# FudanCVL/SynFMC

Measured on AMD Instinct MI355X. Metric: denoising steps/sec, 16x320x512 bf16 U-Net+CMC+OMC, higher is better.
Workload: dtype bf16; 1 GPU; 16x320x512 clip, CFG batch 2, full-width 3D U-Net (1.39B params, random init) + Camera Adapter (CMC) + Object Motion Control (OMC) features, DDIM step; configs/obj.yaml shapes; 1 clip per GPU; frames=16, height=320, width=512, hip_graph=True, fp8_temporal_attention=False, parallelism=dp1 (independent clips, no collective)

## Files before the change

synfmc_amd/csrc/spatial_attn.hip:

```cpp
#include "attn_common.h"
#include <cstdlib>

namespace {

constexpr int SA_WAVES = 4;
constexpr int SA_BQ = 32 * SA_WAVES;
constexpr bool SA_PREFETCH_DEFAULT = true;
constexpr int SA_BK = 64;
constexpr float LOG2E = 1.4426950408889634f;

struct SAParams {
    const void* q; const void* k; const void* v; void* o; float* lse;
    int B, H, Sq, Skv, D;
    int64_t qbs, qrs, kbs, krs, obs, ors;
    int kv_batch_div;
    float scale_log2;
    int nqblk;
    int xcd_remap;
};

constexpr float REF_LIMIT = 64.f;
#ifndef SA_DBG
#define SA_DBG 0
#endif
// ... 826 lines not shown
#pragma unroll
        for (int kb = 0; kb < NKB; ++kb) {
#pragma unroll
            for (int r = 0; r < 16; ++r) s[kb][r] = 0.f;
#pragma unroll
            for (int ks = 0; ks < NKS; ++ks) s[kb] = __builtin_amdgcn_mfma_f32_32x32x16_bf16(kf[kb][ks], qf[ks], s[kb], 0, 0, 0);
        }
        float mx = -INFINITY;
#pragma unroll
        for (int kb = 0; kb < NKB; ++kb)
#pragma unroll
            for (int r = 0; r < 16; ++r) {
                const int key = kb * 32 + (r & 3) + 8 * (r >> 2) + 4 * half;
                if (key >= P.Skv) s[kb][r] = -INFINITY;
                mx = fmaxf(mx, s[kb][r]);
            }
        mx = fmaxf(mx, __shfl_xor(mx, 32, 64));
        f32x16 oacc[NDT];
#pragma unroll
        for (int dt = 0; dt < NDT; ++dt)
#pragma unroll
            for (int r = 0; r < 16; ++r) oacc[dt][r] = 0.f;
#pragma unroll
        for (int kb = 0; kb < NKB; ++kb) {
            float pv[16];
#pragma unroll
            for (int r = 0; r < 16; ++r) pv[r] = __builtin_amdgcn_exp2f(s[kb][r] - mx);
#pragma unroll
            for (int s2 = 0; s2 < 2; ++s2) {
                float p8[8];
#pragma unroll
                for (int i = 0; i < 8; ++i) p8[i] = pv[s2 * 8 + i];
                Frag<bf16_t> pf;
                p_frag(p8, pf);
#pragma unroll
                for (int dt = 0; dt < NDT; ++dt) oacc[dt] = __builtin_amdgcn_mfma_f32_32x32x16_bf16(vf[kb][s2][dt], pf.hi, oacc[dt], 0, 0, 0);
            }
        }
        const float l_tot = __shfl(oacc[NDT - 1][15], l31 + 32, 64);
        const float inv = 1.f / l_tot;
        const int b = kvb * P.kv_batch_div + u / nq32, q = (u - (u / nq32) * nq32) * 32 + l31;
        bf16_t* orow = (bf16_t*)P.o + (int64_t)b * P.obs + (int64_t)q * P.ors + h * D;
#pragma unroll
        for (int dt = 0; dt < NDT; ++dt)
#pragma unroll
            for (int g = 0; g < 4; ++g) {
                const int d = dt * 32 + 8 * g + 4 * half;
                if (d < D)
                    store4<bf16_t>(orow + d, oacc[dt][4 * g] * inv, oacc[dt][4 * g + 1] * inv, oacc[dt][4 * g + 2] * inv, oacc[dt][4 * g + 3] * inv);
            }
        if (P.lse && half == 0) P.lse[((int64_t)b * P.H + h) * P.Sq + q] = mx * 0.6931471805599453f + logf(l_tot);
#pragma unroll
        for (int ks = 0; ks < NKS; ++ks) qf[ks] = qn[ks];
    }
}

inline int sa_xattn_env() {
    static const int v = fmc_env_int("FMC_SA_XATTN", 1);
    return v;
}
inline bool xattn40_ok(const SAParams& P) {
    return P.D == 40 && P.H == 8 && P.Skv <= 96 && P.Skv >= 1 && P.Sq % 32 == 0 && P.B % P.kv_batch_div == 0 && sa_xattn_env() != 0;
}
inline void launch_xattn40(const SAParams& P, hipStream_t st) {
    const int nkvb = P.B / P.kv_batch_div, nq32 = P.Sq / 32, units = P.kv_batch_div * nq32;
    int per = fmc_cu_count() / nkvb;
    if (per < 1) per = 1;
    if (per > units) per = units;
    const size_t lds = (size_t)8 * 96 * XA_VP * 2;
    fmc_launch<xattn40_kernel>(dim3((unsigned)(per * nkvb)), dim3(512), lds, st, P, nq32, units, nkvb);
}

template <int NB>
__global__ __launch_bounds__(320, 1) void sa_small160_kernel(const SAParams P) {
    typedef bf16_t T;
    constexpr int NKS = 10, NDT = 5, KP = NKS * 16 + 8, VPR = sa_vr_pitch<NDT>(), CH = 20, NKEY = NB * 32, NT = 320;
    extern __shared__ __attribute__((aligned(16))) unsigned char smem_raw[];
    T* Ks = reinterpret_cast<T*>(smem_raw);
    T* Vr = Ks + NKEY * KP;
    const int tid = threadIdx.x, lane = tid & 63, wave = tid >> 6;
    const int half = lane >> 5, l31 = lane & 31;
    const int bh = blockIdx.x / P.nqblk, qblk = blockIdx.x - bh * P.nqblk;
    const int b = bh / P.H, h = bh - b * P.H;
    const T* qg = (const T*)P.q + (int64_t)b * P.qbs + (int64_t)h * 160;
    const T* kg = (const T*)P.k + (int64_t)(b / P.kv_batch_div) * P.kbs + (int64_t)h * 160;
    const T* vg = (const T*)P.v + (int64_t)(b / P.kv_batch_div) * P.kbs + (int64_t)h * 160;
    T* og = (T*)P.o + (int64_t)b * P.obs + (int64_t)h * 160;

    constexpr int NSLOT = NKEY * CH / NT;
    static_assert(NKEY * CH % NT == 0, "whole chunks per thread");
    u32x4 kreg[NSLOT], vreg[NSLOT];
    auto gload = [&](const T* base, u32x4 (&reg)[NSLOT]) {
#pragma unroll
        for (int j = 0; j < NSLOT; ++j) {
            const int c = tid + j * NT, row = c / CH, ch = c - row * CH;
            reg[j] = *reinterpret_cast<const u32x4*>(base + (int64_t)(row < P.Skv ? row : P.Skv - 1) * P.krs + ch * 8);
        }
    };
    auto lstore = [&](T* dst, int pitch, const u32x4 (&reg)[NSLOT]) {
#pragma unroll
        for (int j = 0; j < NSLOT; ++j) {
            const int c = tid + j * NT, row = c / CH, ch = c - row * CH;
            *reinterpret_cast<u32x4*>(dst + row * pitch + ch * 8) = reg[j];
        }
    };
    gload(kg, kreg);
    const int qrow = (qblk * 5 + wave) * 32 + l31;
    const bool active = (qblk * 5 + wave) * 32 < P.Sq;
    u32x4 qraw[NKS];
    {
        const T* qp = qg + (int64_t)(qrow < P.Sq ? qrow : P.Sq - 1) * P.qrs + half * 8;
#pragma unroll
        for (int ks = 0; ks < NKS; ++ks) qraw[ks] = *reinterpret_cast<const u32x4*>(qp + ks * 16);
    }
    gload(vg, vreg);
    lstore(Ks, KP, kreg);
    Frag<T> qf[1][NKS];
#pragma unroll
    for (int ks = 0; ks < NKS; ++ks) {
        float qv[8];
#pragma unroll
        for (int i = 0; i < 4; ++i) {
            qv[2 * i] = __uint_as_float(qraw[ks][i] << 16) * P.scale_log2;
            qv[2 * i + 1] = __uint_as_float(qraw[ks][i] & 0xffff0000u) * P.scale_log2;
        }
        p_frag(qv, qf[0][ks]);
    }
    __syncthreads();

    Frag<T> pf[NB][2];
    float m = 0.f, l_run = 0.f;
    if (active) {
        f32x16 s[NB];
#pragma unroll
        for (int blk = 0; blk < NB; ++blk)
#pragma unroll
            for (int r = 0; r < 16; ++r) s[blk][r] = 0.f;
#pragma unroll
        for (int ks = 0; ks < NKS; ++ks)
#pragma unroll
            for (int blk = 0; blk < NB; ++blk) {
                Frag<T> kf;
                make_frag<T>(Ks + (blk * 32 + l31) * KP + ks * 16 + half * 8, kf);
                mma32(kf, qf[0][ks], s[blk]);
            }
        float mx = -INFINITY;
#pragma unroll
        for (int blk = 0; blk < NB; ++blk) {
            if ((blk + 1) * 32 > P.Skv) {
#pragma unroll
                for (int r = 0; r < 16; ++r)
                    if (blk * 32 + (r & 3) + 8 * (r >> 2) + 4 * half >= P.Skv) s[blk][r] = -INFINITY;
            }
            mx = fold_max(s[blk], mx);
        }
        m = fmaxf(mx, __shfl_xor(mx, 32, 64));
#pragma unroll
        for (int blk = 0; blk < NB; ++blk) {
            float p[16];
#pragma unroll
            for (int r = 0; r < 16; ++r) {
                p[r] = __builtin_amdgcn_exp2f(s[blk][r] - m);
                l_run += p[r];
            }
#pragma unroll
            for (int s2 = 0; s2 < 2; ++s2) {
                float p8[8];
#pragma unroll
                for (int i = 0; i < 8; ++i) p8[i] = p[s2 * 8 + i];
                p_frag(p8, pf[blk][s2]);
            }
        }
    }
    lstore(Vr, VPR, vreg);
    __syncthreads();
    if (!active) return;

    f32x16 oacc[NDT];
#pragma unroll
    for (int dt = 0; dt < NDT; ++dt)
#pragma unroll
        for (int r = 0; r < 16; ++r) oacc[dt][r] = 0.f;
#pragma unroll
    for (int blk = 0; blk < NB; ++blk)
#pragma unroll
        for (int s2 = 0; s2 < 2; ++s2)
#pragma unroll
            for (int dt = 0; dt < NDT; ++dt) {
                const T* vp = Vr + (blk * 32 + s2 * 16 + half * 4 + ((l31 & 15) >> 2)) * VPR + dt * 32 + (l31 >> 4) * 16 + (l31 & 3) * 4;
                union { bf16x8 v; sa_s4 hh[2]; } rr;
                rr.hh[0] = lds_tr16(vp);
                rr.hh[1] = lds_tr16(vp + 8 * VPR);
                Frag<T> vf;
                vf.hi = rr.v;
                mma32(vf, pf[blk][s2], oacc[dt]);
            }
    const float l_tot = l_run + __shfl_xor(l_run, 32, 64);
    const float inv = 1.f / l_tot;
    if (qrow < P.Sq) {
        T* orow = og + (int64_t)qrow * P.ors;
#pragma unroll
        for (int dt = 0; dt < NDT; ++dt)
#pragma unroll
            for (int g = 0; g < 4; ++g)
                store4<T>(orow + dt * 32 + 8 * g + 4 * half, oacc[dt][4 * g] * inv, oacc[dt][4 * g + 1] * inv,
                          oacc[dt][4 * g + 2] * inv, oacc[dt][4 * g + 3] * inv);
        if (P.lse && half == 0) P.lse[((int64_t)b * P.H + h) * P.Sq + qrow] = m * 0.6931471805599453f + logf(l_tot);
    }
}

template <int NW>
__device__ __forceinline__ void sa_big80_body(const SAParams& P) {
    typedef bf16_t T;
    constexpr int NKS = 5, NDT = 3, KP = NKS * 16 + 8, VPR = sa_vr_pitch<NDT>(), CH = 10, BKT = NW == 5 ? 160 : 320, NBLK = BKT / 32, NT = 64 * NW;
    extern __shared__ __attribute__((aligned(16))) unsigned char smem_raw[];
    T* Ks = reinterpret_cast<T*>(smem_raw);
    T* Vr = Ks + BKT * KP;
    const int tid = threadIdx.x, lane = tid & 63, wave = tid >> 6;
    const int half = lane >> 5, l31 = lane & 31;
    int bh, qblk;
    {
        const int id = blockIdx.x;
        if (P.xcd_remap == 2) {
            const int xcd = id & 7, within = id >> 3, per_b = P.H * P.nqblk, rem = within % per_b;
            bh = ((within / per_b) * 8 + xcd) * P.H + rem / P.nqblk;
            qblk = rem % P.nqblk;
        } else {
            bh = id / P.nqblk;
            qblk = id - bh * P.nqblk;
        }
    }
    const int b = bh / P.H, h = bh - b * P.H;
    const T* qg = (const T*)P.q + (int64_t)b * P.qbs + (int64_t)h * 80;
    const T* kg = (const T*)P.k + (int64_t)(b / P.kv_batch_div) * P.kbs + (int64_t)h * 80;
    const T* vg = (const T*)P.v + (int64_t)(b / P.kv_batch_div) * P.kbs + (int64_t)h * 80;
    T* og = (T*)P.o + (int64_t)b * P.obs + (int64_t)h * 80;

    constexpr int NSLOT = (BKT * CH + NT - 1) / NT;
    u32x4 kreg[NSLOT], vreg[NSLOT];
    auto gload = [&](int kv0) {
#pragma unroll
        for (int j = 0; j < NSLOT; ++j) {
            const int c = min(tid + j * NT, BKT * CH - 1), row = c / CH, ch = c - row * CH;
            const int kv = kv0 + row < P.Skv ? kv0 + row : P.Skv - 1;
            kreg[j] = *reinterpret_cast<const u32x4*>(kg + (int64_t)kv * P.krs + ch * 8);
            vreg[j] = *reinterpret_cast<const u32x4*>(vg + (int64_t)kv * P.krs + ch * 8);
        }
    };
    auto lstore = [&]() {
#pragma unroll
        for (int j = 0; j < NSLOT; ++j) {
            const int c = min(tid + j * NT, BKT * CH - 1), row = c / CH, ch = c - row * CH;
            *reinterpret_cast<u32x4*>(Ks + row * KP + ch * 8) = kreg[j];
            *reinterpret_cast<u32x4*>(Vr + row * VPR + ch * 8) = vreg[j];
        }
    };
    gload(0);
    const int qrow = (qblk * NW + wave) * 32 + l31;
    const bool active = (qblk * NW + wave) * 32 < P.Sq;
    Frag<T> qf[1][NKS];
    {
        const T* qp = qg + (int64_t)(qrow < P.Sq ? qrow : P.Sq - 1) * P.qrs + half * 8;
        u32x4 qraw[NKS];
#pragma unroll
        for (int ks = 0; ks < NKS; ++ks) qraw[ks] = *reinterpret_cast<const u32x4*>(qp + ks * 16);
#pragma unroll
        for (int ks = 0; ks < NKS; ++ks) {
            float qv[8];
#pragma unroll
            for (int i = 0; i < 4; ++i) {
                qv[2 * i] = __uint_as_float(qraw[ks][i] << 16) * P.scale_log2;
                qv[2 * i + 1] = __uint_as_float(qraw[ks][i] & 0xffff0000u) * P.scale_log2;
            }
            p_frag(qv, qf[0][ks]);
        }
    }
    for (int c = tid; c < BKT * 2; c += NT)
        *reinterpret_cast<u32x4*>(Vr + (c >> 1) * VPR + 80 + (c & 1) * 8) = u32x4{0u, 0u, 0u, (c & 1) ? 0x3f800000u : 0u};
    lstore();
    __syncthreads();

    const int ntiles = (P.Skv + BKT - 1) / BKT;
    float m_ref[1];
    f32x16 negm[1];
    {
        f32x16 zero16;
#pragma unroll
        for (int r = 0; r < 16; ++r) zero16[r] = 0.f;
        const float mx = fold_max(qk_block<T, NKS, false>(Ks, qf[0], zero16, 0, 0, P.Skv, l31, half), -INFINITY);
        m_ref[0] = fmaxf(mx, __shfl_xor(mx, 32, 64));
#pragma unroll
        for (int r = 0; r < 16; ++r) negm[0][r] = -m_ref[0];
    }
    f32x16 oacc[1][NDT];
    float l_run[1];
    for (int pass = 0; pass < 2; ++pass) {
        float worst[1] = {-INFINITY};
#pragma unroll
        for (int dt = 0; dt < NDT; ++dt)
#pragma unroll
            for (int r = 0; r < 16; ++r) oacc[0][dt][r] = 0.f;
        l_run[0] = 0.f;
        for (int tile = 0; tile < ntiles; ++tile) {
#ifndef SA_BIG_DBG
#define SA_BIG_DBG 0
#endif
            if ((tile > 0 || pass > 0) && SA_BIG_DBG != 2) {
                gload(tile * BKT);
                __syncthreads();
                lstore();
                __syncthreads();
            }
            if (active && SA_BIG_DBG != 1) {
                const int nblk = min(NBLK, (P.Skv - tile * BKT) >> 5);
                if (NW == 8 && nblk == NBLK) {
                    f32x16 s[2][1];
                    qk_scores<T, NKS, 1, false>(Ks, qf, negm, s[0], 0, l31, half);
#pragma unroll
                    for (int sb = 0; sb < NBLK; ++sb) {
                        if (sb + 1 < NBLK) qk_scores<T, NKS, 1, false>(Ks, qf, negm, s[(sb + 1) & 1], sb + 1, l31, half);
                        softmax_pv_perq<T, NKS, 1, true>(Vr, s[sb & 1], oacc, worst, l_run, sb, l31, half);
                    }
                } else {
#pragma unroll 1
                    for (int sb = 0; sb < nblk; ++sb)
                        attn_block<T, NKS, 1, false, false, true>(Ks, Vr, qf, oacc, negm, worst, l_run, sb, tile * BKT + sb * 32, P.Skv, l31, half);
                }
            }
        }
        const bool bad = active && worst[0] > REF_LIMIT;
        if (!__syncthreads_or(bad)) break;
        m_ref[0] += fmaxf(worst[0], __shfl_xor(worst[0], 32, 64));
#pragma unroll
        for (int r = 0; r < 16; ++r) negm[0][r] = -m_ref[0];
    }
    if (!active) return;
    const float l_tot = __shfl(oacc[0][NDT - 1][15], l31 + 32, 64);
    const float inv = 1.f / l_tot;
    if (qrow < P.Sq) {
        T* orow = og + (int64_t)qrow * P.ors;
#pragma unroll
        for (int dt = 0; dt < NDT; ++dt)
#pragma unroll
            for (int g = 0; g < 4; ++g) {
                const int d = dt * 32 + 8 * g + 4 * half;
                if (d < 80)
                    store4<T>(orow + d, oacc[0][dt][4 * g] * inv, oacc[0][dt][4 * g + 1] * inv, oacc[0][dt][4 * g + 2] * inv, oacc[0][dt][4 * g + 3] * inv);
            }
        if (P.lse && half == 0) P.lse[((int64_t)b * P.H + h) * P.Sq + qrow] = m_ref[0] * 0.6931471805599453f + logf(l_tot);
    }
}

__global__ __launch_bounds__(640, 1) void sa_big80_kernel_w10(const SAParams P) { sa_big80_body<10>(P); }
__global__ __launch_bounds__(512, 1) void sa_big80_kernel_w8(const SAParams P) { sa_big80_body<8>(P); }
__global__ __launch_bounds__(320, 3) void sa_big80_kernel_w5(const SAParams P) { sa_big80_body<5>(P); }

inline bool sa_big80_ok(const SAParams& P) {
    static const bool on = fmc_env_int("FMC_SA_BIG80", 1) != 0;
    return on && P.D == 80 && P.Skv % 32 == 0 && P.Skv >= 256 && P.Sq >= 160;
}
inline void launch_sa_big80(const SAParams& Pin, hipStream_t st) {
    SAParams P = Pin;
    static const int nw = [] { const int v = fmc_env_int("FMC_SA_BIG80_WAVES", 10); return v == 8 || v == 5 ? v : 10; }();
    P.nqblk = (P.Sq + 32 * nw - 1) / (32 * nw);
    if (P.xcd_remap != 2) P.xcd_remap = 0;
    const size_t lds = (size_t)(nw == 5 ? 160 : 320) * (5 * 16 + 8 + sa_vr_pitch<3>()) * 2;
    if (nw == 5) fmc_launch<sa_big80_kernel_w5>(dim3((unsigned)(P.B * P.H * P.nqblk)), dim3(320), lds, st, P);
    else if (nw == 8) fmc_launch<sa_big80_kernel_w8>(dim3((unsigned)(P.B * P.H * P.nqblk)), dim3(512), lds, st, P);
    else fmc_launch<sa_big80_kernel_w10>(dim3((unsigned)(P.B * P.H * P.nqblk)), dim3(640), lds, st, P);
}

inline bool sa_small_ok(const SAParams& P) {
    static const bool on = fmc_env_int("FMC_SA_SMALL", 1) != 0;
    return on && P.D == 160 && P.Skv <= 160;
}
template <int NB>
void launch_sa_small_nb(const SAParams& P, hipStream_t st) {
    const size_t lds = (size_t)NB * 32 * (10 * 16 + 8 + sa_vr_pitch<5>()) * 2;
    fmc_launch<sa_small160_kernel<NB>>(dim3((unsigned)(P.B * P.H * P.nqblk)), dim3(320), lds, st, P);
}
inline void launch_sa_small(const SAParams& Pin, hipStream_t st) {
    SAParams P = Pin;
    P.nqblk = (P.Sq + 159) / 160;
    if (P.Skv <= 96) launch_sa_small_nb<3>(P, st);
    else launch_sa_small_nb<5>(P, st);
}

inline int sa_pipe_env() {
    static const int v = fmc_env_int("FMC_SA_PIPE", 1);
    return v;
}
inline bool sa40_ok(const SAParams& P) {
    return P.D == 40 && P.Skv % SA_BK == 0 && P.Skv >= 2 * SA_BK && P.Sq % 256 == 0 && P.krs * 2 * (int64_t)P.Skv < (1ll << 31) &&
           sa_pipe_env() != 0;
}
inline void launch_sa40(const SAParams& Pin, hipStream_t st) {
    SAParams P = Pin;
    P.nqblk = P.Sq / 256;
    const int nitems = P.B * P.H * P.nqblk;
    int grid = nitems;
    if (sa_pipe_env() == 4) {
        const int resident = 2 * fmc_cu_count();
        if (nitems > resident) grid = resident;
    }
    hipLaunchKernelGGL(sa40d_kernel, dim3((unsigned)grid), dim3(256), D40_LDS, st, P, nitems);
}

template <typename T, int NKS, bool SHORT_KV, bool PF, int NQ = 1, bool MK = false, bool VR = false>
void launch_sa_v(const SAParams& Pin, hipStream_t st) {
    SAParams P = Pin;
    P.nqblk = (P.Sq + SA_BQ * NQ - 1) / (SA_BQ * NQ);
    constexpr int NDT = (NKS + 1) / 2;
    const size_t lds = sizeof(T) * ((size_t)SA_BK * (NKS * 16 + 8) + (VR ? (size_t)SA_BK * sa_vr_pitch<NDT>() : (size_t)NDT * 32 * (SA_BK + 4)));
    dim3 grid((unsigned)(P.B * P.H * P.nqblk)), block(64 * SA_WAVES);
    fmc_launch<spatial_attn_kernel<T, NKS, SHORT_KV, PF, NQ, MK, VR>>(grid, block, lds, st, P);
}

inline int sa_prefetch_env() {
    static const int v = fmc_env_int("FMC_SA_PREFETCH", -1);
    return v;
}

inline int sa_nq_env() {
    static const int v = fmc_env_int("FMC_SA_NQ", 2);
    return v;
}

inline int sa_vr_env() {
    static const int v = fmc_env_int("FMC_SA_VR", 1);
    return v;
}

inline int sa_mk_env() {
    static const int v = fmc_env_int("FMC_SA_MK", 1);
    return v;
}

template <typename T, int NKS>
void launch_sa(const SAParams& P, hipStream_t st) {
    if (P.Skv <= 2 * SA_BK) {
        if constexpr (sizeof(T) == 2 && NKS <= 6) {
            if (sa_prefetch_env() != 0 && P.Skv > SA_BK) {
                if constexpr (NKS <= 3) {
                    if (sa_nq_env() == 2 && P.Sq >= 2 * SA_BQ) {
                        if (sa_vr_env()) {
                            if (P.D % 16 == 8 && sa_mk_env()) return launch_sa_v<T, NKS, true, true, 2, true, true>(P, st);
                            return launch_sa_v<T, NKS, true, true, 2, false, true>(P, st);
                        }
                        return launch_sa_v<T, NKS, true, true, 2>(P, st);
                    }
                }
                return launch_sa_v<T, NKS, true, true>(P, st);
            }
        }
        launch_sa_v<T, NKS, true, false>(P, st);
    } else {
        if constexpr (sizeof(T) == 2 && NKS <= 6) {
            const int e = sa_prefetch_env();
            if (e < 0 ? SA_PREFETCH_DEFAULT : e != 0) {
                if constexpr (NKS <= 3) {
                    if (sa_nq_env() == 2 && P.Sq >= 2 * SA_BQ) {
                        if (sa_vr_env()) {
                            if (P.D % 16 == 8 && sa_mk_env()) return launch_sa_v<T, NKS, false, true, 2, true, true>(P, st);
                            return launch_sa_v<T, NKS, false, true, 2, false, true>(P, st);
                        }
                        return launch_sa_v<T, NKS, false, true, 2>(P, st);
                    }
                }
                return launch_sa_v<T, NKS, false, true>(P, st);
            }
        }
        launch_sa_v<T, NKS, false, false>(P, st);
    }
}

template <typename T>
int dispatch_sa(const SAParams& P, hipStream_t st) {
    switch ((P.D + 15) / 16) {
        case 1: launch_sa<T, 1>(P, st); break;
        case 2: launch_sa<T, 2>(P, st); break;
        case 3: launch_sa<T, 3>(P, st); break;
        case 4: launch_sa<T, 4>(P, st); break;
        case 5: launch_sa<T, 5>(P, st); break;
        case 6: launch_sa<T, 6>(P, st); break;
        case 8: launch_sa<T, 8>(P, st); break;
        case 10: launch_sa<T, 10>(P, st); break;
        default: FMC_FAIL(FMC_E_SHAPE, "spatial_attn: head dim %d not built (supported: <=96, 113..128, 145..160)", P.D);
    }
    return 0;
}

}

extern "C" int fmc_spatial_attn_fwd(const void* q, const void* k, const void* v, void* o, float* lse, int B, int H,
                                    int Sq, int Skv, int D, int64_t q_batch_stride, int64_t q_row_stride,
                                    int64_t kv_batch_stride, int64_t kv_row_stride, int64_t o_batch_stride,
                                    int64_t o_row_stride, int kv_batch_div, float scale, int dtype, void* stream) {
    if (!q || !k || !v || !o) FMC_FAIL(FMC_E_NULL, "spatial_attn: NULL tensor");
    if (dtype != FMC_BF16 && dtype != FMC_F32) FMC_FAIL(FMC_E_DTYPE, "spatial_attn: dtype %d", dtype);
    if (B <= 0 || H <= 0 || Sq <= 0 || Skv <= 0 || D <= 0 || D % 8 || D > 160 || kv_batch_div <= 0)
        FMC_FAIL(FMC_E_SHAPE, "spatial_attn: need D%%8==0, D<=160, positive sizes (B=%d H=%d Sq=%d Skv=%d D=%d)", B, H, Sq,
                 Skv, D);
    const int64_t strides[] = {q_batch_stride, q_row_stride, kv_batch_stride, kv_row_stride, o_batch_stride, o_row_stride};
    for (int64_t s : strides)
        if (s % 8) FMC_FAIL(FMC_E_ALIGN, "spatial_attn: strides must be multiples of 8 elements");
    if (!fmc_aligned16(q) || !fmc_aligned16(k) || !fmc_aligned16(v) || !fmc_aligned16(o))
        FMC_FAIL(FMC_E_ALIGN, "spatial_attn: tensors must be 16-byte aligned");
    SAParams P;
    P.q = q; P.k = k; P.v = v; P.o = o; P.lse = lse;
    P.B = B; P.H = H; P.Sq = Sq; P.Skv = Skv; P.D = D;
    P.qbs = q_batch_stride; P.qrs = q_row_stride; P.kbs = kv_batch_stride; P.krs = kv_row_stride;
    P.obs = o_batch_stride; P.ors = o_row_stride;
    P.kv_batch_div = kv_batch_div;
    P.scale_log2 = scale * LOG2E;
    P.nqblk = (Sq + SA_BQ - 1) / SA_BQ;
    P.xcd_remap = (B % 8 == 0) ? 2 : ((B * H) % 8 == 0) ? 1 : 0;
    static const int want = fmc_env_int("FMC_SA_XCD", -1);
    if (want == 0 || (want == 1 && (B * H) % 8 == 0)) P.xcd_remap = want;
    hipStream_t st = (hipStream_t)stream;
    if (dtype == FMC_BF16 && xattn40_ok(P)) {
        launch_xattn40(P, st);
        FMC_CHECK_LAUNCH("fmc_spatial_attn_fwd");
        return 0;
    }
    if (dtype == FMC_BF16 && sa_big80_ok(P)) {
        launch_sa_big80(P, st);
        FMC_CHECK_LAUNCH("fmc_spatial_attn_fwd");
        return 0;
    }
    if (dtype == FMC_BF16 && sa_small_ok(P)) {
        launch_sa_small(P, st);
        FMC_CHECK_LAUNCH("fmc_spatial_attn_fwd");
        return 0;
    }
    if (dtype == FMC_BF16 && sa40_ok(P)) {
        launch_sa40(P, st);
        FMC_CHECK_LAUNCH("fmc_spatial_attn_fwd");
        return 0;
    }
    int rc = (dtype == FMC_BF16) ? dispatch_sa<bf16_t>(P, st) : dispatch_sa<float>(P, st);
    if (rc) return rc;
    FMC_CHECK_LAUNCH("fmc_spatial_attn_fwd");
    return 0;
}
```

Baseline: 41.00 steps/s.

## Add software-pipelined D=80 spatial attention kernel with async LDS ring buffers

Adds a new 256-thread spatial attention kernel for head dim 80 that streams K and V tiles straight into LDS ring buffers using buffer_load ... lds. Two waves load K and two load V, and the loop interleaves QK MFMAs, exp2/pack work and PV MFMAs across alternating score buffers. The softmax row sum comes from a constant ones column in V, and the fallback second pass recomputes a max reference only when overflow is detected. The aim is to hide global-load and LDS latency behind MFMA work and to raise occupancy versus the 640-thread kernel. The cost is heavy inline asm, reliance on m0 manipulation, and risk of correctness issues. It also drops the debug macros in the old kernel.

```diff
diff --git a/synfmc_amd/csrc/spatial_attn.hip b/synfmc_amd/csrc/spatial_attn.hip
--- a/synfmc_amd/csrc/spatial_attn.hip
+++ b/synfmc_amd/csrc/spatial_attn.hip
@@ -1152,16 +1152,13 @@
             for (int r = 0; r < 16; ++r) oacc[0][dt][r] = 0.f;
         l_run[0] = 0.f;
         for (int tile = 0; tile < ntiles; ++tile) {
-#ifndef SA_BIG_DBG
-#define SA_BIG_DBG 0
-#endif
-            if ((tile > 0 || pass > 0) && SA_BIG_DBG != 2) {
+            if (tile > 0 || pass > 0) {
                 gload(tile * BKT);
                 __syncthreads();
                 lstore();
                 __syncthreads();
             }
-            if (active && SA_BIG_DBG != 1) {
+            if (active) {
                 const int nblk = min(NBLK, (P.Skv - tile * BKT) >> 5);
                 if (NW == 8 && nblk == NBLK) {
                     f32x16 s[2][1];
@@ -1205,15 +1202,269 @@
 __global__ __launch_bounds__(512, 1) void sa_big80_kernel_w8(const SAParams P) { sa_big80_body<8>(P); }
 __global__ __launch_bounds__(320, 3) void sa_big80_kernel_w5(const SAParams P) { sa_big80_body<5>(P); }
 
+constexpr int P80_RP = 80;
+constexpr int P80_TILE = SA_BK * P80_RP;
+constexpr int P80_VRING = 3 * P80_TILE;
+constexpr int P80_VZERO = 6 * P80_TILE;
+constexpr int P80_VONE = P80_VZERO + 2048;
+constexpr size_t P80_LDS = (size_t)(P80_VONE + 2048) * 2;
+
+__global__ __launch_bounds__(256, 2) void sa_big80_kernel_pipe(const SAParams P) {
+    constexpr int NKS = 5, NDT = 3, D = 80, CH = 10, RP = P80_RP;
+    constexpr int KB_STEP = 32 * RP, VS_STEP = 16 * RP, V8 = 8 * RP;
+    extern __shared__ __attribute__((aligned(16))) unsigned char smem_raw[];
+    bf16_t* smem = reinterpret_cast<bf16_t*>(smem_raw);
+    const int tid = threadIdx.x, lane = tid & 63, wave = __builtin_amdgcn_readfirstlane(tid >> 6);
+    const int half = lane >> 5, l31 = lane & 31;
+
+    for (int i = tid; i < 2048; i += 256) {
+        smem[P80_VZERO + i] = (bf16_t)0;
+        smem[P80_VONE + i] = ((i & 3) == 3) ? f2bf(1.f) : (bf16_t)0;
+    }
+
+    int bh, qblk;
+    {
+        const int id = blockIdx.x;
+        if (P.xcd_remap == 2) {
+            const int xcd = id & 7, within = id >> 3, per_b = P.H * P.nqblk, rem = within % per_b;
+            bh = ((within / per_b) * 8 + xcd) * P.H + rem / P.nqblk;
+            qblk = rem % P.nqblk;
+        } else {
+            bh = id / P.nqblk;
+            qblk = id - bh * P.nqblk;
+        }
+    }
+    const int b = bh / P.H, h = bh - b * P.H;
+    const bf16_t* qg = (const bf16_t*)P.q + (int64_t)b * P.qbs + (int64_t)h * D;
+    const bf16_t* kg = (const bf16_t*)P.k + (int64_t)(b / P.kv_batch_div) * P.kbs + (int64_t)h * D;
+    const bf16_t* vg = (const bf16_t*)P.v + (int64_t)(b / P.kv_batch_div) * P.kbs + (int64_t)h * D;
+    bf16_t* og = (bf16_t*)P.o + (int64_t)b * P.obs + (int64_t)h * D;
+
+    const int qrow = (qblk * SA_WAVES + wave) * 32 + l31;
+    u32x4 qraw[NKS];
+    {
+        const bf16_t* qp = qg + (int64_t)(qrow < P.Sq ? qrow : P.Sq - 1) * P.qrs + half * 8;
+#pragma unroll
+        for (int ks = 0; ks < NKS; ++ks) qraw[ks] = *reinterpret_cast<const u32x4*>(qp + ks * 16);
+    }
+
+    const bool isK = wave < 2;
+    const int krsB = (int)P.krs * 2, tile_bytes = SA_BK * krsB;
+    const int kv_bytes = (int)(((int64_t)(P.Skv - 1) * P.krs + D) * 2);
+    const int ntiles = P.Skv / SA_BK;
+    const __amdgpu_buffer_rsrc_t rs = __builtin_amdgcn_make_buffer_rsrc((void*)(isK ? kg : vg), 0, kv_bytes, 0x00020000);
+    unsigned vo[5];
+#pragma unroll
+    for (int i = 0; i < 5; ++i) {
+        const int c = ((wave & 1) * 5 + i) * 64 + lane, row = c / CH, ch = c - row * CH;
+        const int key = isK ? row : (row & ~15) + 8 * ((row >> 3) & 1) + 4 * (row & 1) + ((row >> 1) & 3);
+        vo[i] = (unsigned)(key * krsB + (isK ? (ch ^ ((row >> 3) & 1)) : ch) * 16);
+    }
+    const int piece0 = (wave & 1) * 5 * 512;
+    auto stage = [&](int tile, bf16_t* dst) {
+        const int so = (tile < ntiles ? tile : ntiles - 1) * tile_bytes;
+        const unsigned lds = (unsigned)(uintptr_t)(__attribute__((address_space(3))) bf16_t*)(dst + piece0);
+        unsigned keep;
+        asm volatile("s_nop 4\n\ts_mov_b32 %0, m0\n\ts_mov_b32 m0, %7\n\ts_nop 0\n\t"
+                     "buffer_load_dwordx4 %1, %6, %8 offen lds\n\ts_add_u32 m0, m0, 0x400\n\ts_nop 0\n\t"
+                     "buffer_load_dwordx4 %2, %6, %8 offen lds\n\ts_add_u32 m0, m0, 0x400\n\ts_nop 0\n\t"
+                     "buffer_load_dwordx4 %3, %6, %8 offen lds\n\ts_add_u32 m0, m0, 0x400\n\ts_nop 0\n\t"
+                     "buffer_load_dwordx4 %4, %6, %8 offen lds\n\ts_add_u32 m0, m0, 0x400\n\ts_nop 0\n\t"
+                     "buffer_load_dwordx4 %5, %6, %8 offen lds\n\ts_mov_b32 m0, %0"
+                     : "=&s"(keep)
+                     : "v"(vo[0]), "v"(vo[1]), "v"(vo[2]), "v"(vo[3]), "v"(vo[4]), "s"(rs), "s"(lds), "s"(so)
+                     : "memory", "scc");
+    };
+    auto ring = [&](int i3) { return smem + (isK ? 0 : P80_VRING) + i3 * P80_TILE; };
+
+    const int ka = l31 * RP + (half ^ ((l31 >> 3) & 1)) * 8;
+    const int va = (half + 2 * ((l31 & 15) >> 2)) * RP + (l31 >> 4) * 16 + (l31 & 3) * 4;
+    const bool vdata = (l31 >> 4) == 0;
+    const bf16_t* vconst = smem + ((l31 & 3) == 3 ? P80_VONE + 4 : P80_VZERO) + (half ? 0 : 16);
+
+    bf16x8 kf[NKS], vf[2][NDT];
+    auto kload = [&](const bf16_t* kp, int ks) { kf[ks] = lds_frag(kp + ks * 16); };
+    auto vload = [&](const bf16_t* vp, const bf16_t* vp2, int s2, int dt) {
+        const bf16_t* p = dt == 2 ? vp2 : vp + dt * 32;
+        union { bf16x8 v; sa_s4 h[2]; } r;
+        r.h[0] = lds_tr16(p + s2 * VS_STEP); r.h[1] = lds_tr16(p + s2 * VS_STEP + V8);
+        vf[s2][dt] = r.v;
+    };
+    auto kptr = [&](const bf16_t* buf, int kb) { return buf + ka + kb * KB_STEP; };
+    auto vptr = [&](const bf16_t* buf, int kb) { return buf + va + kb * 2 * VS_STEP; };
+    auto vptr2 = [&](const bf16_t* buf, int kb) { return vdata ? buf + va + kb * 2 * VS_STEP + 64 : vconst; };
+
+    __syncthreads();
+    auto request_first = [&] {
+        stage(0, ring(0)); stage(1, ring(1));
+        if (isK) stage(2, ring(2));
+    };
+    request_first();
+    bf16x8 qf[NKS];
+    {
+#pragma unroll
+        for (int ks = 0; ks < NKS; ++ks) {
+            float qv[8];
+#pragma unroll
+            for (int i = 0; i < 4; ++i) {
+                qv[2 * i] = __uint_as_float(qraw[ks][i] << 16) * P.scale_log2;
+                qv[2 * i + 1] = __uint_as_float(qraw[ks][i] & 0xffff0000u) * P.scale_log2;
+            }
+            Frag<bf16_t> f;
+            p_frag(qv, f);
+            qf[ks] = f.hi;
+        }
+    }
+    float m_ref = 0.f;
+    f32x16 negm;
+#pragma unroll
+    for (int r = 0; r < 16; ++r) negm[r] = 0.f;
+    auto scores = [&]() {
+        f32x16 sacc = negm;
+#pragma unroll
+        for (int ks = 0; ks < NKS; ++ks) sacc = __builtin_amdgcn_mfma_f32_32x32x16_bf16(kf[ks], qf[ks], sacc, 0, 0, 0);
+        return sacc;
+    };
+    auto set_ref = [&](float m) {
+        m_ref = m;
+#pragma unroll
+        for (int r = 0; r < 16; ++r) negm[r] = -m;
+    };
+
+    f32x16 oacc[NDT];
+    for (int pass = 0; pass < 2; ++pass) {
+        if (pass == 1) { __syncthreads(); request_first(); }
+        asm volatile("s_waitcnt vmcnt(5)" ::: "memory");
+        __syncthreads();
+        const bf16_t* K0 = smem;
+        const bf16_t* V0 = smem + P80_VRING;
+#pragma unroll
+        for (int ks = 0; ks < NKS; ++ks) kload(kptr(K0, 0), ks);
+        if (pass == 0) {
+            const float mx = fold_max(scores(), -INFINITY);
+            set_ref(fmaxf(mx, __shfl_xor(mx, 32, 64)));
+        }
+#pragma unroll
+        for (int dt = 0; dt < NDT; ++dt)
+#pragma unroll
+            for (int r = 0; r < 16; ++r) oacc[dt][r] = 0.f;
+
+        f32x16 sA = scores(), sB;
+        PFrag pA[2], pB[2];
+#pragma unroll
+        for (int ks = 0; ks < NKS; ++ks) kload(kptr(K0, 1), ks);
+#pragma unroll
+        for (int s2 = 0; s2 < 2; ++s2) {
+#pragma unroll
+            for (int dt = 0; dt < NDT; ++dt) vload(vptr(V0, 0), vptr2(V0, 0), s2, dt);
+#pragma unroll
+            for (int i = 0; i < 4; ++i) pB[s2].u[i] = 0u;
+        }
+
+        auto step = [&](const f32x16& sS, PFrag (&pS)[2], f32x16& sQ, const PFrag (&pP)[2], const bf16_t* kN, const bf16_t* vN,
+                        const bf16_t* vN2, auto&& head) {
+            float e[16];
+            auto QK = [&](int ks) {
+                P40_SB();
+                sQ = __builtin_amdgcn_mfma_f32_32x32x16_bf16(kf[ks], qf[ks], ks == 0 ? negm : sQ, 0, 0, 0);
+                P40_SB();
+                kload(kN, ks);
+            };
+            auto PV = [&](int s2, int dt) {
+                P40_SB();
+                oacc[dt] = __builtin_amdgcn_mfma_f32_32x32x16_bf16(vf[s2][dt], as_frag(pP[s2]), oacc[dt], 0, 0, 0);
+                P40_SB();
+                vload(vN, vN2, s2, dt);
+            };
+            auto EX = [&](int i) { e[i] = __builtin_amdgcn_exp2f(sS[i]); };
+            auto PK = [&](int j) { pS[j >> 2].u[j & 3] = pack_bf2(e[2 * j], e[2 * j + 1]); };
+            P40_SB();
+            head();
+            QK(0);    EX(0); EX(1);
+            PV(0, 0); PK(0); EX(2);
+            QK(1);    EX(3); PK(1); EX(4);
+            PV(0, 1); EX(5); PK(2);
+            QK(2);    EX(6); EX(7);
+            PV(0, 2); PK(3); EX(8);
+            QK(3);    EX(9); PK(4); EX(10);
+            PV(1, 0); EX(11); PK(5);
+            QK(4);    EX(12); EX(13);
+            PV(1, 1); PK(6); EX(14);
+            PV(1, 2); EX(15); PK(7);
+            P40_SB();
+        };
+
+        int i3 = 0;
+        for (int t = 0; t < ntiles; ++t) {
+            const int n3 = i3 == 2 ? 0 : i3 + 1, p3 = i3 == 0 ? 2 : i3 - 1;
+            const bf16_t* Kn = smem + n3 * P80_TILE;
+            const bf16_t* Vc = smem + P80_VRING + i3 * P80_TILE;
+            step(sA, pA, sB, pB, kptr(Kn, 0), vptr(Vc, 0), vptr2(Vc, 0), [&] {
+                asm volatile("s_waitcnt vmcnt(5) lgkmcnt(0)\n\ts_barrier" ::: "memory");
+                stage(t + (isK ? 3 : 2), ring(isK ? i3 : p3));
+            });
+            step(sB, pB, sA, pA, kptr(Kn, 1), vptr(Vc, 1), vptr2(Vc, 1), [] {});
+            i3 = n3;
+        }
+#pragma unroll
+        for (int s2 = 0; s2 < 2; ++s2)
+#pragma unroll
+            for (int dt = 0; dt < NDT; ++dt)
+                oacc[dt] = __builtin_amdgcn_mfma_f32_32x32x16_bf16(vf[s2][dt], as_frag(pB[s2]), oacc[dt], 0, 0, 0);
+        asm volatile("s_waitcnt vmcnt(0)" ::: "memory");
+
+        const bool bad = half == 1 && oacc[NDT - 1][15] > 1.8446744e19f;
+        if (pass == 1 || !__syncthreads_or(bad)) break;
+        float worst = -INFINITY;
+        for (int t = 0; t < ntiles; ++t) {
+            __syncthreads();
+            if (isK) stage(t, smem);
+            asm volatile("s_waitcnt vmcnt(0)" ::: "memory");
+            __syncthreads();
+#pragma unroll
+            for (int kb = 0; kb < 2; ++kb) {
+#pragma unroll
+                for (int ks = 0; ks < NKS; ++ks) kload(kptr(smem, kb), ks);
+                worst = fold_max(scores(), worst);
+            }
+        }
+        set_ref(m_ref + fmaxf(worst, __shfl_xor(worst, 32, 64)));
+    }
+
+    const float l_tot = __shfl(oacc[NDT - 1][15], l31 + 32, 64);
+    const float inv = 1.f / l_tot;
+    if (qrow < P.Sq) {
+        bf16_t* orow = og + (int64_t)qrow * P.ors;
+#pragma unroll
+        for (int dt = 0; dt < NDT; ++dt)
+#pragma unroll
+            for (int g = 0; g < 4; ++g) {
+                const int d = dt * 32 + 8 * g + 4 * half;
+                if (d < D)
+                    store4<bf16_t>(orow + d, oacc[dt][4 * g] * inv, oacc[dt][4 * g + 1] * inv, oacc[dt][4 * g + 2] * inv, oacc[dt][4 * g + 3] * inv);
+            }
+        if (P.lse && half == 0) P.lse[((int64_t)b * P.H + h) * P.Sq + qrow] = m_ref * 0.6931471805599453f + logf(l_tot);
+    }
+}
+
 inline bool sa_big80_ok(const SAParams& P) {
     static const bool on = fmc_env_int("FMC_SA_BIG80", 1) != 0;
     return on && P.D == 80 && P.Skv % 32 == 0 && P.Skv >= 256 && P.Sq >= 160;
 }
+inline bool sa_big80_pipe_ok(const SAParams& P) {
+    static const bool on = fmc_env_int("FMC_SA_BIG80_PIPE", 1) != 0 && std::getenv("FMC_SA_BIG80_WAVES") == nullptr;
+    return on && P.Skv % SA_BK == 0 && P.krs * 2 * (int64_t)P.Skv < (1ll << 31);
+}
 inline void launch_sa_big80(const SAParams& Pin, hipStream_t st) {
     SAParams P = Pin;
+    if (P.xcd_remap != 2) P.xcd_remap = 0;
+    if (sa_big80_pipe_ok(P)) {
+        P.nqblk = (P.Sq + SA_BQ - 1) / SA_BQ;
+        fmc_launch<sa_big80_kernel_pipe>(dim3((unsigned)(P.B * P.H * P.nqblk)), dim3(256), P80_LDS, st, P);
+        return;
+    }
     static const int nw = [] { const int v = fmc_env_int("FMC_SA_BIG80_WAVES", 10); return v == 8 || v == 5 ? v : 10; }();
     P.nqblk = (P.Sq + 32 * nw - 1) / (32 * nw);
-    if (P.xcd_remap != 2) P.xcd_remap = 0;
     const size_t lds = (size_t)(nw == 5 ? 160 : 320) * (5 * 16 + 8 + sa_vr_pitch<3>()) * 2;
     if (nw == 5) fmc_launch<sa_big80_kernel_w5>(dim3((unsigned)(P.B * P.H * P.nqblk)), dim3(320), lds, st, P);
     else if (nw == 8) fmc_launch<sa_big80_kernel_w8>(dim3((unsigned)(P.B * P.H * P.nqblk)), dim3(512), lds, st, P);
```

New measurement: 41.00 steps/s. No clear change (-0.0%).
